# risc0/RustCrypto-elliptic-curves

Measured on AMD Instinct MI355X. Metric: k256 variable-base scalar-muls/sec, higher is better.
Workload: dtype u32

## Files before the change

__graft_entry__.py:

```python
import os
import subprocess
import sys

ROOT = os.path.dirname(os.path.abspath(__file__))
PKG = os.path.join(ROOT, "rustcrypto-elliptic-curves_amd")
for p in (ROOT, PKG):
    if p not in sys.path:
        sys.path.insert(0, p)


def build() -> None:
    env = dict(os.environ)
    env.setdefault("HIPCC", "/opt/rocm/bin/hipcc")
    subprocess.run(["make", "-j%d" % max(2, min(8, os.cpu_count() or 4)), "-C", PKG], check=True, env=env)
    oracle_dir = os.path.join(ROOT, "oracle")
    if os.path.exists(os.path.join(oracle_dir, "Makefile")):
        subprocess.run(["make", "-C", oracle_dir], check=True, env=env)
    subprocess.run(["make", "-C", os.path.join(ROOT, "tools", "ubench"), "libecpeak.so"], check=True, env=env)
    subprocess.run(["make", "-C", os.path.join(ROOT, "examples")], check=True, env=env)
    subprocess.run(["make", "-C", os.path.join(ROOT, "tests", "hosttwin")], check=True, env=env)
    subprocess.run(["make", "-j3", "-C", os.path.join(ROOT, "tests", "devtwin")], check=True, env=env)
    import ecgpu
    ecgpu.load_library()


def smoke() -> None:
    import numpy as np
    import ecgpu
    from oracle import ecmodel as M
    from oracle import synth

    ctx = ecgpu.Context(0)
    c = M.K256
    cv = ctx.curve("k256")
    n = 64
    ks = synth.scalars(c, n)
    ps = synth.points(c, n)
    sb = np.frombuffer(b"".join(M.i2b(c, k) for k in ks), dtype=np.uint8).reshape(n, 32).copy()
    pb = np.frombuffer(b"".join(M.i2b(c, x) + M.i2b(c, y) for x, y in ps), dtype=np.uint8).reshape(n, 64).copy()
    xy, inf = cv.mul(sb, pb)
    for i in range(n):
        w = M.affine_mul(c, ks[i], ps[i])
        assert bytes(xy[i]) == M.i2b(c, w[0]) + M.i2b(c, w[1]) and inf[i] == 0, f"k256 mul mismatch at {i}"
    xyz = cv.mul(sb, pb, out_format=ecgpu.PROJECTIVE, flags=ecgpu.EXACT_REFERENCE)
    for i in range(0, n, 8):
        assert bytes(xyz[i]) == M.proj_bytes(c, M.k256_mul_ref((ps[i][0], ps[i][1], 1), ks[i])), f"exact XYZ mismatch at {i}"
    ctx.close()
    print("smoke ok: k256 variable-base scalar multiplication on cuda:0 is bit-exact against the oracle")


if __name__ == "__main__":
    build()
    if len(sys.argv) > 1 and sys.argv[1] == "smoke":
        smoke()
```

rustcrypto-elliptic-curves_amd/csrc/fe_k256.hpp:

```cpp
#pragma once
#include "mp32.hpp"

namespace ecgpu {

struct FeK256 {
  static constexpr int N = 8;
  static constexpr int NBYTES = 32;
  u32 v[8];
};

namespace k256 {

static constexpr u32 C_LO = 977;

#ifdef ECGPU_K256_BRANCHFREE
#define ECGPU_K256_RARE(cond) true
#else
#define ECGPU_K256_RARE(cond) __builtin_expect((cond), 0)
#endif
#if defined(ECGPU_K256_BRANCHFREE) || defined(ECGPU_K256_EXACT_PRODUCTS)
#define ECGPU_K256_SPEC_PRODUCTS 0
#else
#define ECGPU_K256_SPEC_PRODUCTS 1
#endif

ECGPU_HD void fold_top(u32* r, u64 T) {
  const u64 m = (u64)(u32)T * C_LO + (((u64)((u32)(T >> 32) * C_LO)) << 32);
  const u64 alo = m + (T << 32);
  const u32 a2 = (u32)(T >> 32) + (alo < m ? 1u : 0u);
  u32 c = 0;
  r[0] = addc(r[0], (u32)alo, c);
  r[1] = addc(r[1], (u32)(alo >> 32), c);
  r[2] = addc(r[2], a2, c);
#pragma unroll
  for (int i = 3; i < 8; i++) r[i] = addc(r[i], 0u, c);
  u32 c2 = 0;
  r[0] = addc(r[0], c ? C_LO : 0u, c2);
  r[1] = addc(r[1], c, c2);
  r[2] = addc(r[2], 0u, c2);
}

ECGPU_HD void fold_top_fast(u32* r, u64 T) {
  const u32 t0 = (u32)T, t1 = (u32)(T >> 32);
  const u64 p = (u64)t0 * C_LO;
  const u32 s1 = (u32)(p >> 32) + t1 * C_LO;
  u32 ca = 0;
  const u32 a1 = addc(s1, t0, ca);
  const u32 a2 = t1 + ca;
  u32 c = 0;
  r[0] = addc(r[0], (u32)p, c);
  r[1] = addc(r[1], a1, c);
  r[2] = addc(r[2], a2, c);
  if (ECGPU_K256_RARE(c != 0)) {
#pragma unroll
    for (int i = 3; i < 8; i++) r[i] = addc(r[i], 0u, c);
    u32 c2 = 0;
    r[0] = addc(r[0], c ? C_LO : 0u, c2);
    r[1] = addc(r[1], c, c2);
    r[2] = addc(r[2], 0u, c2);
  }
}

namespace nc_bound {
using u128 = unsigned __int128;
constexpr u128 MAX_PRODUCT = (u128)0xFFFFFFFFu * 0xFFFFFFFFu;
static_assert(17 * MAX_PRODUCT + ((u128)1 << 37) < ((u128)1 << 69), "a column with a carry-in < 2^37 sums to < 2^69: it pops < 2^37");
static_assert(((u128)1 << 37) + (u128)0xFFFFFFFFu * C_LO < ((u128)1 << 43), "fold product on a popped carry: < 2^43, no carry");
static_assert(((u128)1 << 37) + 0xFFFFFFFFu < ((u128)1 << 64), "s_i * d_8 on a popped carry: no carry");
static_assert((u128)0xFFFFFFFFu + MAX_PRODUCT < ((u128)1 << 64), "s_0 * d_8 then one product on a zeroed accumulator: no carry");
}
template <int K>
ECGPU_HD void mul_high_column(u32* h, Acc96& c, const u32* a, const u32* b) {
  mac_product_column<8, K, 0, true, (K == 8 ? 1 : 0)>(c, a, b, nullptr, nullptr);
  h[K - 8] = acc_pop(c);
}
template <int K>
ECGPU_HD void mul_low_column(u32* t, Acc96& c, const u32* a, const u32* b, const u32* h) {
  const u32 xa[1] = {h[K]}, xb[1] = {C_LO};
  mac_product_column<8, K, 1, true, 1>(c, a, b, xa, xb);
  t[K] = acc_pop(c);
}
ECGPU_HD void mul_exact(FeK256& r, const FeK256& a, const FeK256& b) {
  u32 h[8], t[8];
  Acc96 c{0, 0};
  mul_high_column<8>(h, c, a.v, b.v);  mul_high_column<9>(h, c, a.v, b.v);
  mul_high_column<10>(h, c, a.v, b.v); mul_high_column<11>(h, c, a.v, b.v);
  mul_high_column<12>(h, c, a.v, b.v); mul_high_column<13>(h, c, a.v, b.v);
  mul_high_column<14>(h, c, a.v, b.v);
  h[7] = (u32)c.lo;
  c.lo = 0; c.hi = 0;
  mul_low_column<0>(t, c, a.v, b.v, h); mul_low_column<1>(t, c, a.v, b.v, h);
  mul_low_column<2>(t, c, a.v, b.v, h); mul_low_column<3>(t, c, a.v, b.v, h);
  mul_low_column<4>(t, c, a.v, b.v, h); mul_low_column<5>(t, c, a.v, b.v, h);
  mul_low_column<6>(t, c, a.v, b.v, h); mul_low_column<7>(t, c, a.v, b.v, h);
  u32 cy = 0;
  r.v[0] = t[0];
#pragma unroll
  for (int i = 1; i < 8; i++) r.v[i] = addc(t[i], h[i - 1], cy);
  const u64 T = c.lo + h[7] + cy;
  fold_top_fast(r.v, T);
}

namespace nc_bound {
constexpr u128 high_carry_in(int K) {
  u128 c = 0;
  for (int k = 8; k < K; k++) c = (c + (u128)(15 - k) * MAX_PRODUCT) >> 32;
  return c;
}
static_assert(high_carry_in(14) + MAX_PRODUCT < ((u128)1 << 64), "mul, high column 14: a_7 b_7 on the popped carry cannot carry");
static_assert(2 * high_carry_in(14) + 1 + MAX_PRODUCT >= ((u128)1 << 64), "with two products per column (mul_add2) it can: speculative there");
static_assert(((u128)1 << 43) + MAX_PRODUCT >= ((u128)1 << 64) && MAX_PRODUCT == ((u128)1 << 64) - ((u128)1 << 33) + 1,
              "low half: the speculative product starts below 2^43 and carries only for a product above 2^64 - 2^43");
static_assert(((u128)1 << 37) + 0xFFFFFFFFu < ((u128)1 << 38), "high half: the speculative product starts below 2^38 (popped carry, + s_i d_8 in mul_add_sqr)");
}
#if !ECGPU_K256_SPEC_PRODUCTS
ECGPU_HD void mul(FeK256& r, const FeK256& a, const FeK256& b) { mul_exact(r, a, b); }
#else
template <int K>
ECGPU_HD void mul_high_column_spec(u32* h, Acc96& c, const u32* a, const u32* b, u64& raised) {
  static_assert(K >= 9 && K <= 14, "column 8 starts from zero and stays mul_high_column<8>");
  if constexpr (K == 14) {
    mac_nc(c, a[7], b[7]);
    h[6] = (u32)c.lo;
    c.lo >>= 32;
    return;
  } else {
    u64 k = 0;
    mac_product_column<8, K, 0, true, 0, true>(c, a, b, nullptr, nullptr, k);
    ECGPU_SPEC_NOTE("mul", K, k != 0);
    raised |= k;
  }
  h[K - 8] = acc_pop(c);
}
template <int K>
ECGPU_HD void mul_low_column_spec(u32* t, Acc96& c, const u32* a, const u32* b, const u32* h, u64& raised) {
  static_assert(K >= 1 && K <= 7, "column 0 has one product after the fold term, whose carry addition creates c.hi: it stays mul_low_column<0>");
  const u32 xa[1] = {h[K]}, xb[1] = {C_LO};
  u64 k = 0;
  mac_product_column<8, K, 1, true, 1, true>(c, a, b, xa, xb, k);
  ECGPU_SPEC_NOTE("mul", K, k != 0);
  raised |= k;
  t[K] = acc_pop(c);
}
ECGPU_HD void mul_finish(FeK256& r, const u32* t, const u32* h, const Acc96& c, u32 h8) {
  u32 cy = 0;
  r.v[0] = t[0];
#pragma unroll
  for (int i = 1; i < 8; i++) r.v[i] = addc(t[i], h[i - 1], cy);
  const u64 T = c.lo + h[7] + cy + (((u64)h8 << 32) | (h8 ? C_LO : 0u));
  fold_top_fast(r.v, T);
}
ECGPU_HD void mul(FeK256& r, const FeK256& a, const FeK256& b) {
  u32 h[8], t[8];
  u64 raised = 0;
  Acc96 c{0, 0};
  mul_high_column<8>(h, c, a.v, b.v);
  mul_high_column_spec<9>(h, c, a.v, b.v, raised);  mul_high_column_spec<10>(h, c, a.v, b.v, raised);
  mul_high_column_spec<11>(h, c, a.v, b.v, raised); mul_high_column_spec<12>(h, c, a.v, b.v, raised);
  mul_high_column_spec<13>(h, c, a.v, b.v, raised); mul_high_column_spec<14>(h, c, a.v, b.v, raised);
  h[7] = (u32)c.lo;
  c.lo = 0; c.hi = 0;
  mul_low_column<0>(t, c, a.v, b.v, h); mul_low_column_spec<1>(t, c, a.v, b.v, h, raised);
  mul_low_column_spec<2>(t, c, a.v, b.v, h, raised); mul_low_column_spec<3>(t, c, a.v, b.v, h, raised);
  mul_low_column_spec<4>(t, c, a.v, b.v, h, raised); mul_low_column_spec<5>(t, c, a.v, b.v, h, raised);
  mul_low_column_spec<6>(t, c, a.v, b.v, h, raised); mul_low_column_spec<7>(t, c, a.v, b.v, h, raised);
  mul_finish(r, t, h, c, 0);
}
#endif

template <int K>
ECGPU_HD void mul2_high_column(u32* h, Acc96& c, const u32* a, const u32* b, const u32* e, const u32* f) {
  mac_product_column<8, K, 0, true, (K == 8 ? 1 : 0)>(c, a, b, nullptr, nullptr);
  mac_product_column<8, K, 0, false>(c, e, f, nullptr, nullptr);
  h[K - 8] = acc_pop(c);
}
template <int K>
ECGPU_HD void mul2_low_column(u32* t, Acc96& c, const u32* a, const u32* b, const u32* e, const u32* f, const u32* h) {
  const u32 xa[1] = {h[K]}, xb[1] = {C_LO};
  mac_product_column<8, K, 1, true, 1>(c, a, b, xa, xb);
  mac_product_column<8, K, 0, false>(c, e, f, nullptr, nullptr);
  t[K] = acc_pop(c);
}
ECGPU_HD void mul_add2_exact(FeK256& r, const FeK256& a, const FeK256& b, const FeK256& e, const FeK256& f) {
  u32 h[8], t[8];
  Acc96 c{0, 0};
  mul2_high_column<8>(h, c, a.v, b.v, e.v, f.v);  mul2_high_column<9>(h, c, a.v, b.v, e.v, f.v);
  mul2_high_column<10>(h, c, a.v, b.v, e.v, f.v); mul2_high_column<11>(h, c, a.v, b.v, e.v, f.v);
  mul2_high_column<12>(h, c, a.v, b.v, e.v, f.v); mul2_high_column<13>(h, c, a.v, b.v, e.v, f.v);
  mul2_high_column<14>(h, c, a.v, b.v, e.v, f.v);
  h[7] = (u32)c.lo;
  const u32 h8 = (u32)(c.lo >> 32);
  c.lo = 0; c.hi = 0;
  mul2_low_column<0>(t, c, a.v, b.v, e.v, f.v, h); mul2_low_column<1>(t, c, a.v, b.v, e.v, f.v, h);
  mul2_low_column<2>(t, c, a.v, b.v, e.v, f.v, h); mul2_low_column<3>(t, c, a.v, b.v, e.v, f.v, h);
  mul2_low_column<4>(t, c, a.v, b.v, e.v, f.v, h); mul2_low_column<5>(t, c, a.v, b.v, e.v, f.v, h);
  mul2_low_column<6>(t, c, a.v, b.v, e.v, f.v, h); mul2_low_column<7>(t, c, a.v, b.v, e.v, f.v, h);
  u32 cy = 0;
  r.v[0] = t[0];
#pragma unroll
  for (int i = 1; i < 8; i++) r.v[i] = addc(t[i], h[i - 1], cy);
  const u64 T = c.lo + h[7] + cy + (((u64)h8 << 32) | (h8 ? C_LO : 0u));
  fold_top_fast(r.v, T);
}

#if !ECGPU_K256_SPEC_PRODUCTS
ECGPU_HD void mul_add2(FeK256& r, const FeK256& a, const FeK256& b, const FeK256& e, const FeK256& f) { mul_add2_exact(r, a, b, e, f); }
#else
template <int K>
ECGPU_HD void mul2_high_column_spec(u32* h, Acc96& c, const u32* a, const u32* b, const u32* e, const u32* f, u64& raised) {
  static_assert(K >= 9 && K <= 13, "column 8 starts from zero; column 14 has one product a_7 b_7, whose carry addition creates c.hi");
  u64 k = 0;
  mac_product_column<8, K, 0, true, 0, true>(c, a, b, nullptr, nullptr, k);
  ECGPU_SPEC_NOTE("mul_add2", K, k != 0);
  raised |= k;
  mac_product_column<8, K, 0, false>(c, e, f, nullptr, nullptr);
  h[K - 8] = acc_pop(c);
}
template <int K>
ECGPU_HD void mul2_low_column_spec(u32* t, Acc96& c, const u32* a, const u32* b, const u32* e, const u32* f, const u32* h, u64& raised) {
  static_assert(K >= 1 && K <= 7, "column 0 stays mul2_low_column<0>, as in mul");
  const u32 xa[1] = {h[K]}, xb[1] = {C_LO};
  u64 k = 0;
  mac_product_column<8, K, 1, true, 1, true>(c, a, b, xa, xb, k);
  ECGPU_SPEC_NOTE("mul_add2", K, k != 0);
  raised |= k;
  mac_product_column<8, K, 0, false>(c, e, f, nullptr, nullptr);
  t[K] = acc_pop(c);
}
ECGPU_HD void mul_add2(FeK256& r, const FeK256& a, const FeK256& b, const FeK256& e, const FeK256& f) {
  u32 h[8], t[8];
  u64 raised = 0;
  Acc96 c{0, 0};
  mul2_high_column<8>(h, c, a.v, b.v, e.v, f.v);
  mul2_high_column_spec<9>(h, c, a.v, b.v, e.v, f.v, raised);  mul2_high_column_spec<10>(h, c, a.v, b.v, e.v, f.v, raised);
  mul2_high_column_spec<11>(h, c, a.v, b.v, e.v, f.v, raised); mul2_high_column_spec<12>(h, c, a.v, b.v, e.v, f.v, raised);
  mul2_high_column_spec<13>(h, c, a.v, b.v, e.v, f.v, raised); mul2_high_column<14>(h, c, a.v, b.v, e.v, f.v);
  h[7] = (u32)c.lo;
  const u32 h8 = (u32)(c.lo >> 32);
  c.lo = 0; c.hi = 0;
  mul2_low_column<0>(t, c, a.v, b.v, e.v, f.v, h); mul2_low_column_spec<1>(t, c, a.v, b.v, e.v, f.v, h, raised);
  mul2_low_column_spec<2>(t, c, a.v, b.v, e.v, f.v, h, raised); mul2_low_column_spec<3>(t, c, a.v, b.v, e.v, f.v, h, raised);
  mul2_low_column_spec<4>(t, c, a.v, b.v, e.v, f.v, h, raised); mul2_low_column_spec<5>(t, c, a.v, b.v, e.v, f.v, h, raised);
  mul2_low_column_spec<6>(t, c, a.v, b.v, e.v, f.v, h, raised); mul2_low_column_spec<7>(t, c, a.v, b.v, e.v, f.v, h, raised);
  mul_finish(r, t, h, c, h8);
}
#endif

constexpr int sqr2_terms(int K) {
  int m = 0;
  if (K % 2 == 1 && (K - 1) / 2 <= 6) m++;
  if (K % 2 == 0 && K / 2 <= 7) m++;
  for (int i = 0; i <= 6; i++)
    if (K - i >= i + 2 && K - i <= 8) m++;
  return m;
}
constexpr bool sqr2_has_d8(int K) { return K >= 8 && K <= 14; }
template <int K>
ECGPU_HD void sqr2_column_terms(u32* pa, u32* pb, const u32* s, const u32* e, const u32* d) {
  int m = 0;
  if constexpr (K % 2 == 1 && (K - 1) / 2 <= 6) { pa[m] = s[(K - 1) / 2]; pb[m] = e[(K + 1) / 2]; m++; }
  if constexpr (K % 2 == 0 && K / 2 <= 7) { pa[m] = s[K / 2]; pb[m] = s[K / 2]; m++; }
#pragma unroll
  for (int i = 0; i <= 6; i++)
    if (K - i >= i + 2 && K - i <= 7) { pa[m] = s[i]; pb[m] = d[K - i]; m++; }
}
ECGPU_HD void sqr2_operands(u32* e, u32* d, const u32* s) {
#pragma unroll
  for (int j = 1; j < 8; j++) e[j] = s[j] << 1;
#pragma unroll
  for (int j = 2; j < 8; j++) d[j] = (s[j] << 1) | (s[j - 1] >> 31);
  d[8] = s[7] >> 31;
}
template <int K, int NX, bool FRESH, int NC>
ECGPU_HD void mulsq_column(Acc96& c, const u32* a, const u32* b, const u32* s, const u32* e, const u32* d, const u32* xa, const u32* xb) {
  constexpr int LO = (K - 7) > 0 ? (K - 7) : 0;
  constexpr int HI = K < 7 ? K : 7;
  constexpr int M = HI - LO + 1;
  constexpr int MS = sqr2_terms(K);
  constexpr int D8 = sqr2_has_d8(K) ? 1 : 0;
  u32 pa[M + MS + NX + 1], pb[M + MS + NX + 1];
#pragma unroll
  for (int m = 0; m < NX; m++) { pa[m] = xa[m]; pb[m] = xb[m]; }
  if constexpr (D8) { pa[NX] = s[K - 8]; pb[NX] = d[8]; }
#pragma unroll
  for (int m = 0; m < M; m++) { pa[NX + D8 + m] = a[LO + m]; pb[NX + D8 + m] = b[K - LO - m]; }
  sqr2_column_terms<K>(pa + NX + D8 + M, pb + NX + D8 + M, s, e, d);
  mac_cols<M + MS + NX, FRESH, NC>(c, pa, pb);
}
template <int K>
ECGPU_HD void mulsq_high_column(u32* h, Acc96& c, const u32* a, const u32* b, const u32* s, const u32* e, const u32* d) {
  static_assert(sqr2_has_d8(K), "every high column has its d_8 term");
  mulsq_column<K, 0, true, (K == 8 ? 2 : 1)>(c, a, b, s, e, d, nullptr, nullptr);
  h[K - 8] = acc_pop(c);
}
template <int K>
ECGPU_HD void mulsq_low_column(u32* t, Acc96& c, const u32* a, const u32* b, const u32* s, const u32* e, const u32* d, const u32* h) {
  const u32 xa[1] = {h[K]}, xb[1] = {C_LO};
  mulsq_column<K, 1, true, 1>(c, a, b, s, e, d, xa, xb);
  t[K] = acc_pop(c);
}
ECGPU_HD void mul_add_sqr_exact(FeK256& r, const FeK256& a, const FeK256& b, const FeK256& s) {
  u32 e[8], d[9], h[8], t[8];
  e[0] = 0; d[0] = 0; d[1] = 0;
  sqr2_operands(e, d, s.v);
  Acc96 c{0, 0};
  mulsq_high_column<8>(h, c, a.v, b.v, s.v, e, d);  mulsq_high_column<9>(h, c, a.v, b.v, s.v, e, d);
  mulsq_high_column<10>(h, c, a.v, b.v, s.v, e, d); mulsq_high_column<11>(h, c, a.v, b.v, s.v, e, d);
  mulsq_high_column<12>(h, c, a.v, b.v, s.v, e, d); mulsq_high_column<13>(h, c, a.v, b.v, s.v, e, d);
  mulsq_high_column<14>(h, c, a.v, b.v, s.v, e, d);
  h[7] = (u32)c.lo;
  const u32 h8 = (u32)(c.lo >> 32);
  c.lo = 0; c.hi = 0;
  mulsq_low_column<0>(t, c, a.v, b.v, s.v, e, d, h); mulsq_low_column<1>(t, c, a.v, b.v, s.v, e, d, h);
  mulsq_low_column<2>(t, c, a.v, b.v, s.v, e, d, h); mulsq_low_column<3>(t, c, a.v, b.v, s.v, e, d, h);
  mulsq_low_column<4>(t, c, a.v, b.v, s.v, e, d, h); mulsq_low_column<5>(t, c, a.v, b.v, s.v, e, d, h);
  mulsq_low_column<6>(t, c, a.v, b.v, s.v, e, d, h); mulsq_low_column<7>(t, c, a.v, b.v, s.v, e, d, h);
  u32 cy = 0;
  r.v[0] = t[0];
#pragma unroll
  for (int i = 1; i < 8; i++) r.v[i] = addc(t[i], h[i - 1], cy);
  const u64 T = c.lo + h[7] + cy + (((u64)h8 << 32) | (h8 ? C_LO : 0u));
  fold_top_fast(r.v, T);
}

#if !ECGPU_K256_SPEC_PRODUCTS
ECGPU_HD void mul_add_sqr(FeK256& r, const FeK256& a, const FeK256& b, const FeK256& s) { mul_add_sqr_exact(r, a, b, s); }
#else
template <int K, int NX, int NC>
ECGPU_HD void mulsq_column_spec(Acc96& c, const u32* a, const u32* b, const u32* s, const u32* e, const u32* d, const u32* xa, const u32* xb, u64& raised) {
  constexpr int LO = (K - 7) > 0 ? (K - 7) : 0;
  constexpr int HI = K < 7 ? K : 7;
  constexpr int M = HI - LO + 1;
  constexpr int MS = sqr2_terms(K);
  constexpr int D8 = sqr2_has_d8(K) ? 1 : 0;
  u32 pa[M + MS + NX + 1], pb[M + MS + NX + 1];
#pragma unroll
  for (int m = 0; m < NX; m++) { pa[m] = xa[m]; pb[m] = xb[m]; }
  if constexpr (D8) { pa[NX] = s[K - 8]; pb[NX] = d[8]; }
#pragma unroll
  for (int m = 0; m < M; m++) { pa[NX + D8 + m] = a[LO + m]; pb[NX + D8 + m] = b[K - LO - m]; }
  sqr2_column_terms<K>(pa + NX + D8 + M, pb + NX + D8 + M, s, e, d);
  u64 k = 0;
  mac_cols<M + MS + NX, true, NC, true>(c, pa, pb, k);
  ECGPU_SPEC_NOTE("mul_add_sqr", K, k != 0);
  raised |= k;
}
template <int K>
ECGPU_HD void mulsq_high_column_spec(u32* h, Acc96& c, const u32* a, const u32* b, const u32* s, const u32* e, const u32* d, u64& raised) {
  static_assert(K >= 9 && K <= 14, "column 8 starts from zero and stays mulsq_high_column<8>");
  mulsq_column_spec<K, 0, 1>(c, a, b, s, e, d, nullptr, nullptr, raised);
  h[K - 8] = acc_pop(c);
}
template <int K>
ECGPU_HD void mulsq_low_column_spec(u32* t, Acc96& c, const u32* a, const u32* b, const u32* s, const u32* e, const u32* d, const u32* h, u64& raised) {
  const u32 xa[1] = {h[K]}, xb[1] = {C_LO};
  mulsq_column_spec<K, 1, 1>(c, a, b, s, e, d, xa, xb, raised);
  t[K] = acc_pop(c);
}
ECGPU_HD void mul_add_sqr(FeK256& r, const FeK256& a, const FeK256& b, const FeK256& s) {
  u32 e[8], d[9], h[8], t[8];
  e[0] = 0; d[0] = 0; d[1] = 0;
  sqr2_operands(e, d, s.v);
  u64 raised = 0;
  Acc96 c{0, 0};
  mulsq_high_column<8>(h, c, a.v, b.v, s.v, e, d);
  mulsq_high_column_spec<9>(h, c, a.v, b.v, s.v, e, d, raised);  mulsq_high_column_spec<10>(h, c, a.v, b.v, s.v, e, d, raised);
  mulsq_high_column_spec<11>(h, c, a.v, b.v, s.v, e, d, raised); mulsq_high_column_spec<12>(h, c, a.v, b.v, s.v, e, d, raised);
  mulsq_high_column_spec<13>(h, c, a.v, b.v, s.v, e, d, raised); mulsq_high_column_spec<14>(h, c, a.v, b.v, s.v, e, d, raised);
  h[7] = (u32)c.lo;
  const u32 h8 = (u32)(c.lo >> 32);
  c.lo = 0; c.hi = 0;
  mulsq_low_column_spec<0>(t, c, a.v, b.v, s.v, e, d, h, raised); mulsq_low_column_spec<1>(t, c, a.v, b.v, s.v, e, d, h, raised);
  mulsq_low_column_spec<2>(t, c, a.v, b.v, s.v, e, d, h, raised); mulsq_low_column_spec<3>(t, c, a.v, b.v, s.v, e, d, h, raised);
  mulsq_low_column_spec<4>(t, c, a.v, b.v, s.v, e, d, h, raised); mulsq_low_column_spec<5>(t, c, a.v, b.v, s.v, e, d, h, raised);
  mulsq_low_column_spec<6>(t, c, a.v, b.v, s.v, e, d, h, raised); mulsq_low_column_spec<7>(t, c, a.v, b.v, s.v, e, d, h, raised);
  mul_finish(r, t, h, c, h8);
}
#endif

ECGPU_HD void reduce16(FeK256& r, const u32* w) {
  u32 u[8];
  u64 acc = 0;
#pragma unroll
  for (int k = 0; k < 8; k++) {
    acc = (u64)w[8 + k] * C_LO + (acc >> 32);
    u[k] = (u32)acc;
  }
  u32 c1 = 0, c2 = 0;
  u32 t[8];
#pragma unroll
  for (int k = 0; k < 8; k++) t[k] = addc(w[k], u[k], c1);
  r.v[0] = t[0];
#pragma unroll
  for (int k = 1; k < 8; k++) r.v[k] = addc(t[k], w[8 + k - 1], c2);
  const u64 T = (acc >> 32) + c1 + c2 + w[15];
  fold_top_fast(r.v, T);
}

ECGPU_HD void sqr_exact(FeK256& r, const FeK256& a) {
  u32 w[16];
  mp_sqr_wide<8>(w, a.v);
  reduce16(r, w);
}

ECGPU_HD void sqr(FeK256& r, const FeK256& a) {
#if !ECGPU_K256_SPEC_PRODUCTS
  sqr_exact(r, a);
#else
  u32 w[16];
  u64 raised = 0;
  mp_sqr_wide<8, true>(w, a.v, raised);
  reduce16(r, w);
#endif
}

ECGPU_HD void add(FeK256& r, const FeK256& a, const FeK256& b) {
  const u32 c = mp_add<8>(r.v, a.v, b.v);
  u32 c2 = 0;
  r.v[0] = addc(r.v[0], c ? C_LO : 0u, c2);
  r.v[1] = addc(r.v[1], c, c2);
  if (ECGPU_K256_RARE(c2 != 0)) {
#pragma unroll
    for (int i = 2; i < 8; i++) r.v[i] = addc(r.v[i], 0u, c2);
    u32 c3 = 0;
    r.v[0] = addc(r.v[0], c2 ? C_LO : 0u, c3);
    r.v[1] = addc(r.v[1], c2, c3);
  }
}

ECGPU_HD void sub(FeK256& r, const FeK256& a, const FeK256& b) {
  const u32 bw = mp_sub<8>(r.v, a.v, b.v);
  u32 b2 = 0;
  r.v[0] = subb(r.v[0], bw ? C_LO : 0u, b2);
  r.v[1] = subb(r.v[1], bw, b2);
  if (ECGPU_K256_RARE(b2 != 0)) {
#pragma unroll
    for (int i = 2; i < 8; i++) r.v[i] = subb(r.v[i], 0u, b2);
    u32 b3 = 0;
    r.v[0] = subb(r.v[0], b2 ? C_LO : 0u, b3);
    r.v[1] = subb(r.v[1], b2, b3);
  }
}

ECGPU_HD void sub2(FeK256& r, const FeK256& a, const FeK256& b, const FeK256& c) {
  const u32 w = mp_sub<8>(r.v, a.v, b.v) + mp_sub<8>(r.v, r.v, c.v);
  u32 b2 = 0;
  r.v[0] = subb(r.v[0], w * C_LO, b2);
  r.v[1] = subb(r.v[1], w, b2);
  if (ECGPU_K256_RARE(b2 != 0)) {
#pragma unroll
    for (int i = 2; i < 8; i++) r.v[i] = subb(r.v[i], 0u, b2);
    u32 b3 = 0;
    r.v[0] = subb(r.v[0], b2 ? C_LO : 0u, b3);
    r.v[1] = subb(r.v[1], b2, b3);
  }
}

ECGPU_HD void half(FeK256& r, const FeK256& a) {
  const u32 m = 0u - (a.v[0] & 1u);
  u32 t[8], c = 0;
  t[0] = addc(a.v[0], m & (0u - C_LO), c);
  t[1] = addc(a.v[1], m & 0xFFFFFFFEu, c);
#pragma unroll
  for (int i = 2; i < 8; i++) t[i] = addc(a.v[i], m, c);
#pragma unroll
  for (int i = 0; i < 7; i++) r.v[i] = (t[i] >> 1) | (t[i + 1] << 31);
  r.v[7] = (t[7] >> 1) | (c << 31);
}

ECGPU_HD void set_zero(FeK256& r) { mp_zero<8>(r.v); }
ECGPU_HD void set_one(FeK256& r) { mp_zero<8>(r.v); r.v[0] = 1; }
ECGPU_HD void set_u32(FeK256& r, u32 x) { mp_zero<8>(r.v); r.v[0] = x; }

ECGPU_HD void neg(FeK256& r, const FeK256& a) {
  FeK256 z;
  set_zero(z);
  sub(r, z, a);
}
ECGPU_HD void dbl(FeK256& r, const FeK256& a) { add(r, a, a); }

template <int K>
ECGPU_HD void shl(FeK256& r, const FeK256& a) {
  static_assert(K >= 1 && K <= 3, "small shifts only");
  const u32 top = a.v[7] >> (32 - K);
  u32 t[8];
#pragma unroll
  for (int i = 7; i >= 1; i--) t[i] = (a.v[i] << K) | (a.v[i - 1] >> (32 - K));
  t[0] = a.v[0] << K;
  u32 c = 0;
  r.v[0] = addc(t[0], top * C_LO, c);
  r.v[1] = addc(t[1], top, c);
#pragma unroll
  for (int i = 2; i < 8; i++) r.v[i] = t[i];
  if (ECGPU_K256_RARE(c != 0)) {
// ... 115 lines not shown
```

rustcrypto-elliptic-curves_amd/csrc/mp32.hpp:

```cpp
#pragma once
#include <stdint.h>

#if defined(__HIPCC__)
#include <hip/hip_runtime.h>
#define ECGPU_HD __host__ __device__ __forceinline__
#else
#define ECGPU_HD inline
#endif

#if defined(__HIP_DEVICE_COMPILE__)
#define ECGPU_ASM 1
#else
#define ECGPU_ASM 0
#endif

#ifndef ECGPU_TABLE_TOUCH
#define ECGPU_TABLE_TOUCH(idx) ((void)0)
#endif
#ifndef ECGPU_EXC_NOTE
#define ECGPU_EXC_NOTE(site, cond) ((void)0)
#endif
#ifndef ECGPU_SPEC_NOTE
#define ECGPU_SPEC_NOTE(site, column, raised) ((void)0)
#endif
// ... 76 lines not shown
template <int N>
ECGPU_HD void mp_select(u32* r, bool cond, const u32* a, const u32* b) {
#pragma unroll
  for (int i = 0; i < N; i++) r[i] = cond ? a[i] : b[i];
}

struct Acc96 {
  u64 lo;
  u32 hi;
};

ECGPU_HD void mac(Acc96& c, u32 a, u32 b) {
#if ECGPU_ASM
  asm("v_mad_u64_u32 %0, vcc, %2, %3, %0\n\tv_addc_co_u32 %1, vcc, 0, %1, vcc"
      : "+v"(c.lo), "+v"(c.hi)
      : "v"(a), "v"(b)
      : "vcc");
#else
  u64 p = (u64)a * b;
  c.lo += p;
  c.hi += (c.lo < p);
#endif
}
ECGPU_HD void mac_nc(Acc96& c, u32 a, u32 b) { c.lo += (u64)a * b; }
ECGPU_HD u64 mac_spec(Acc96& c, u32 a, u32 b) {
  const u64 p = (u64)a * b;
  c.lo += p;
  return c.lo < p ? 1u : 0u;
}
ECGPU_HD void mac_spec_fix(Acc96& c, u64 k) {
#if ECGPU_ASM
  asm("v_addc_co_u32 %0, vcc, 0, %0, %1" : "+v"(c.hi) : "s"(k) : "vcc");
#else
  c.hi += (u32)k;
#endif
}
ECGPU_HD void acc_sub32(Acc96& c, u32 w) {
  u32 l0 = (u32)c.lo, l1 = (u32)(c.lo >> 32), bw = 0;
  l0 = subb(l0, w, bw);
  l1 = subb(l1, 0u, bw);
  c.hi = subb(c.hi, 0u, bw);
  c.lo = ((u64)l1 << 32) | l0;
}

#include "mp32_cols.inc"

template <int M, bool FRESH = false, int NC = 0>
ECGPU_HD void mac_cols(Acc96& c, const u32* pa, const u32* pb) {
  static_assert(M >= 1, "column length");
  static_assert(NC >= 0 && NC <= 2 && NC <= M, "at most two leading products without a carry");
  if constexpr (M > 12) {
    mac_cols<12, FRESH, NC>(c, pa, pb);
    mac_cols<M - 12, false>(c, pa + 12, pb + 12);
  } else if constexpr (NC > 0) {
    mac_cols_nc<M, FRESH, NC>(c, pa, pb);
  } else {
    if constexpr (M == 1) { if constexpr (FRESH) mac_col1_f(c, pa[0], pb[0]); else mac_col1(c, pa[0], pb[0]); }
    if constexpr (M == 2) { if constexpr (FRESH) mac_col2_f(c, pa[0], pb[0], pa[1], pb[1]); else mac_col2(c, pa[0], pb[0], pa[1], pb[1]); }
    if constexpr (M == 3) { if constexpr (FRESH) mac_col3_f(c, pa[0], pb[0], pa[1], pb[1], pa[2], pb[2]); else mac_col3(c, pa[0], pb[0], pa[1], pb[1], pa[2], pb[2]); }
    if constexpr (M == 4) { if constexpr (FRESH) mac_col4_f(c, pa[0], pb[0], pa[1], pb[1], pa[2], pb[2], pa[3], pb[3]); else mac_col4(c, pa[0], pb[0], pa[1], pb[1], pa[2], pb[2], pa[3], pb[3]); }
    if constexpr (M == 5) { if constexpr (FRESH) mac_col5_f(c, pa[0], pb[0], pa[1], pb[1], pa[2], pb[2], pa[3], pb[3], pa[4], pb[4]); else mac_col5(c, pa[0], pb[0], pa[1], pb[1], pa[2], pb[2], pa[3], pb[3], pa[4], pb[4]); }
    if constexpr (M == 6) { if constexpr (FRESH) mac_col6_f(c, pa[0], pb[0], pa[1], pb[1], pa[2], pb[2], pa[3], pb[3], pa[4], pb[4], pa[5], pb[5]); else mac_col6(c, pa[0], pb[0], pa[1], pb[1], pa[2], pb[2], pa[3], pb[3], pa[4], pb[4], pa[5], pb[5]); }
    if constexpr (M == 7) { if constexpr (FRESH) mac_col7_f(c, pa[0], pb[0], pa[1], pb[1], pa[2], pb[2], pa[3], pb[3], pa[4], pb[4], pa[5], pb[5], pa[6], pb[6]); else mac_col7(c, pa[0], pb[0], pa[1], pb[1], pa[2], pb[2], pa[3], pb[3], pa[4], pb[4], pa[5], pb[5], pa[6], pb[6]); }
    if constexpr (M == 8) { if constexpr (FRESH) mac_col8_f(c, pa[0], pb[0], pa[1], pb[1], pa[2], pb[2], pa[3], pb[3], pa[4], pb[4], pa[5], pb[5], pa[6], pb[6], pa[7], pb[7]); else mac_col8(c, pa[0], pb[0], pa[1], pb[1], pa[2], pb[2], pa[3], pb[3], pa[4], pb[4], pa[5], pb[5], pa[6], pb[6], pa[7], pb[7]); }
    if constexpr (M == 9) { if constexpr (FRESH) mac_col9_f(c, pa[0], pb[0], pa[1], pb[1], pa[2], pb[2], pa[3], pb[3], pa[4], pb[4], pa[5], pb[5], pa[6], pb[6], pa[7], pb[7], pa[8], pb[8]); else mac_col9(c, pa[0], pb[0], pa[1], pb[1], pa[2], pb[2], pa[3], pb[3], pa[4], pb[4], pa[5], pb[5], pa[6], pb[6], pa[7], pb[7], pa[8], pb[8]); }
    if constexpr (M == 10) { if constexpr (FRESH) mac_col10_f(c, pa[0], pb[0], pa[1], pb[1], pa[2], pb[2], pa[3], pb[3], pa[4], pb[4], pa[5], pb[5], pa[6], pb[6], pa[7], pb[7], pa[8], pb[8], pa[9], pb[9]); else mac_col10(c, pa[0], pb[0], pa[1], pb[1], pa[2], pb[2], pa[3], pb[3], pa[4], pb[4], pa[5], pb[5], pa[6], pb[6], pa[7], pb[7], pa[8], pb[8], pa[9], pb[9]); }
    if constexpr (M == 11) { if constexpr (FRESH) mac_col11_f(c, pa[0], pb[0], pa[1], pb[1], pa[2], pb[2], pa[3], pb[3], pa[4], pb[4], pa[5], pb[5], pa[6], pb[6], pa[7], pb[7], pa[8], pb[8], pa[9], pb[9], pa[10], pb[10]); else mac_col11(c, pa[0], pb[0], pa[1], pb[1], pa[2], pb[2], pa[3], pb[3], pa[4], pb[4], pa[5], pb[5], pa[6], pb[6], pa[7], pb[7], pa[8], pb[8], pa[9], pb[9], pa[10], pb[10]); }
    if constexpr (M == 12) { if constexpr (FRESH) mac_col12_f(c, pa[0], pb[0], pa[1], pb[1], pa[2], pb[2], pa[3], pb[3], pa[4], pb[4], pa[5], pb[5], pa[6], pb[6], pa[7], pb[7], pa[8], pb[8], pa[9], pb[9], pa[10], pb[10], pa[11], pb[11]); else mac_col12(c, pa[0], pb[0], pa[1], pb[1], pa[2], pb[2], pa[3], pb[3], pa[4], pb[4], pa[5], pb[5], pa[6], pb[6], pa[7], pb[7], pa[8], pb[8], pa[9], pb[9], pa[10], pb[10], pa[11], pb[11]); }
  }
}
template <int M, bool FRESH = false, int NC = 0, bool SPEC = false>
ECGPU_HD void mac_cols(Acc96& c, const u32* pa, const u32* pb, u64& raised) {
  if constexpr (!SPEC) {
    mac_cols<M, FRESH, NC>(c, pa, pb);
  } else {
    static_assert(M >= 1 && NC >= 0 && NC <= 2 && NC + 1 <= M, "the speculative product follows the no-carry products");
    u64 k;
    if constexpr (M > 12) {
      mac_cols_s1<12, FRESH, NC>(c, k, pa, pb);
      mac_cols<M - 12, false>(c, pa + 12, pb + 12);
    } else {
      mac_cols_s1<M, FRESH, NC>(c, k, pa, pb);
    }
    if (__builtin_expect(k != 0, 0)) mac_spec_fix(c, k);
    raised |= k;
  }
}
template <int N, int K, int NX, bool FRESH = false, int NC = 0>
ECGPU_HD void mac_product_column(Acc96& c, const u32* a, const u32* b, const u32* xa, const u32* xb) {
  constexpr int LO = (K - (N - 1)) > 0 ? (K - (N - 1)) : 0;
  constexpr int HI = K < (N - 1) ? K : (N - 1);
  constexpr int M = HI - LO + 1;
  u32 pa[M + NX + 1], pb[M + NX + 1];
#pragma unroll
  for (int m = 0; m < NX; m++) { pa[m] = xa[m]; pb[m] = xb[m]; }
#pragma unroll
  for (int m = 0; m < M; m++) { pa[NX + m] = a[LO + m]; pb[NX + m] = b[K - LO - m]; }
  mac_cols<M + NX, FRESH, NC>(c, pa, pb);
}
template <int N, int K, int NX, bool FRESH = false, int NC = 0, bool SPEC = false>
ECGPU_HD void mac_product_column(Acc96& c, const u32* a, const u32* b, const u32* xa, const u32* xb, u64& raised) {
  constexpr int LO = (K - (N - 1)) > 0 ? (K - (N - 1)) : 0;
  constexpr int HI = K < (N - 1) ? K : (N - 1);
  constexpr int M = HI - LO + 1;
  u32 pa[M + NX + 1], pb[M + NX + 1];
#pragma unroll
  for (int m = 0; m < NX; m++) { pa[m] = xa[m]; pb[m] = xb[m]; }
#pragma unroll
  for (int m = 0; m < M; m++) { pa[NX + m] = a[LO + m]; pb[NX + m] = b[K - LO - m]; }
  mac_cols<M + NX, FRESH, NC, SPEC>(c, pa, pb, raised);
}

ECGPU_HD u32 acc_pop(Acc96& c) {
  u32 r = (u32)c.lo;
  c.lo = (c.lo >> 32) | ((u64)c.hi << 32);
  c.hi = 0;
  return r;
}

ECGPU_HD u32 acc_pop_signed(Acc96& c) {
  u32 r = (u32)c.lo;
  c.lo = (c.lo >> 32) | ((u64)c.hi << 32);
  c.hi = (u32)((int32_t)c.hi >> 31);
  return r;
}

template <int N>
ECGPU_HD void mp_mul_wide(u32* r, const u32* a, const u32* b) {
  Acc96 c{0, 0};
#pragma unroll
  for (int k = 0; k < 2 * N - 1; k++) {
#pragma unroll
    for (int i = 0; i < N; i++) {
      const int j = k - i;
      if (j >= 0 && j < N) {
        if (k == 0 || k == 2 * N - 2) mac_nc(c, a[i], b[j]); else mac(c, a[i], b[j]);
      }
    }
    r[k] = acc_pop(c);
  }
  r[2 * N - 1] = (u32)c.lo;
}


template <int N, int K>
ECGPU_HD void mac_cross_column(Acc96& c, const u32* a) {
  constexpr int LO = (K - (N - 1)) > 0 ? (K - (N - 1)) : 0;
  constexpr int HI = (K - 1) / 2;
  constexpr int M = HI - LO + 1;
  if constexpr (M >= 1) {
    u32 pa[M], pb[M];
#pragma unroll
    for (int m = 0; m < M; m++) { pa[m] = a[LO + m]; pb[m] = a[K - LO - m]; }
    mac_cols<M, true>(c, pa, pb);
  }
}
template <int N, int K>
ECGPU_HD void sqr_cross_columns(u32* x, Acc96& c, const u32* a) {
  if constexpr (K < 2 * N - 2) {
    mac_cross_column<N, K>(c, a);
    x[K] = acc_pop(c);
    sqr_cross_columns<N, K + 1>(x, c, a);
  }
}

template <int N>
constexpr bool sqr_cross_first_nc(int K) {
  typedef unsigned __int128 u128;
  const u128 maxp = (u128)0xFFFFFFFFu * 0xFFFFFFFFu;
  u128 c = 0;
  for (int k = 1; k < K; k++) {
    const int lo = (k - (N - 1)) > 0 ? (k - (N - 1)) : 0, hi = (k - 1) / 2;
    c = (c + (u128)(hi - lo + 1) * maxp) >> 32;
  }
  return c + maxp < ((u128)1 << 64);
}
static_assert(sqr_cross_first_nc<8>(1) && sqr_cross_first_nc<8>(2) && sqr_cross_first_nc<8>(3) && sqr_cross_first_nc<8>(4) && sqr_cross_first_nc<8>(5) &&
              !sqr_cross_first_nc<8>(6) && !sqr_cross_first_nc<8>(10) && sqr_cross_first_nc<8>(11) && sqr_cross_first_nc<8>(12) && sqr_cross_first_nc<8>(13),
              "the carry-free cross columns of the 8-word square, as the comments and tests/k256_spec_carry_vectors.py list them");
template <int N, int K, bool SPEC>
ECGPU_HD void mac_cross_column(Acc96& c, const u32* a, u64& raised) {
  constexpr int LO = (K - (N - 1)) > 0 ? (K - (N - 1)) : 0;
  constexpr int HI = (K - 1) / 2;
  constexpr int M = HI - LO + 1;
  if constexpr (M >= 1) {
    u32 pa[M], pb[M];
#pragma unroll
    for (int m = 0; m < M; m++) { pa[m] = a[LO + m]; pb[m] = a[K - LO - m]; }
    if constexpr (SPEC && M == 1 && sqr_cross_first_nc<N>(K)) mac_nc(c, pa[0], pb[0]);
    else if constexpr (SPEC && M >= 2 && sqr_cross_first_nc<N>(K)) mac_cols<M, true, 1>(c, pa, pb);
    else mac_cols<M, true, 0, (SPEC && M >= 2)>(c, pa, pb, raised);
  }
}
template <int N, int K, bool SPEC>
ECGPU_HD void sqr_cross_columns(u32* x, Acc96& c, const u32* a, u64& raised) {
  if constexpr (K < 2 * N - 2) {
    u64 k = 0;
    mac_cross_column<N, K, SPEC>(c, a, k);
    if constexpr (SPEC && (K - 1) / 2 - ((K - (N - 1)) > 0 ? (K - (N - 1)) : 0) + 1 >= 2 && !sqr_cross_first_nc<N>(K)) { ECGPU_SPEC_NOTE("sqr", K, k != 0); }
    raised |= k;
    x[K] = acc_pop(c);
    sqr_cross_columns<N, K + 1, SPEC>(x, c, a, raised);
  }
}

template <int N>
ECGPU_HD void mp_sqr_wide(u32* r, const u32* a) {
  u32 x[2 * N];
  Acc96 c{0, 0};
  x[0] = 0;
  sqr_cross_columns<N, 1>(x, c, a);
  x[2 * N - 2] = (u32)c.lo;
  x[2 * N - 1] = (u32)(c.lo >> 32);
  u32 carry = 0;
#pragma unroll
  for (int i = 0; i < N; i++) {
    const u64 d = (u64)a[i] * a[i];
    const u32 lo2 = (x[2 * i] << 1) | (i ? (x[2 * i - 1] >> 31) : 0);
    const u32 hi2 = (x[2 * i + 1] << 1) | (x[2 * i] >> 31);
    r[2 * i] = addc(lo2, (u32)d, carry);
    r[2 * i + 1] = addc(hi2, (u32)(d >> 32), carry);
  }
}
template <int N, bool SPEC>
ECGPU_HD void mp_sqr_wide(u32* r, const u32* a, u64& raised) {
  u32 x[2 * N];
  Acc96 c{0, 0};
  x[0] = 0;
  sqr_cross_columns<N, 1, SPEC>(x, c, a, raised);
  x[2 * N - 2] = (u32)c.lo;
  x[2 * N - 1] = (u32)(c.lo >> 32);
  u32 carry = 0;
#pragma unroll
  for (int i = 0; i < N; i++) {
    const u64 d = (u64)a[i] * a[i];
    const u32 lo2 = (x[2 * i] << 1) | (i ? (x[2 * i - 1] >> 31) : 0);
    const u32 hi2 = (x[2 * i + 1] << 1) | (x[2 * i] >> 31);
    r[2 * i] = addc(lo2, (u32)d, carry);
    r[2 * i + 1] = addc(hi2, (u32)(d >> 32), carry);
  }
}

ECGPU_HD u32 bswap32(u32 x) { return __builtin_bswap32(x); }

}
```

Before: 160.2 million.

## Replace per-column speculative carry fixups with whole-product recompute on rare miss

Previously each speculative product column tested its raised-carry mask and applied mac_spec_fix inline. Now each multiply, multiply-add and square first runs all columns without fixups. If any column raised a carry, it reruns the whole product with fixups enabled, and the rare branch is marked with probability 1.0 so it is laid out cold. This removes per-column branches and fixup code from the hot path, in exchange for a full recompute on a mispredicted carry and larger code.

Measured after the change: 161.6 million, median of 6. No clear change (+0.9%).

```diff
diff --git a/__graft_entry__.py b/__graft_entry__.py
--- a/__graft_entry__.py
+++ b/__graft_entry__.py
@@ -20,6 +20,7 @@
     subprocess.run(["make", "-C", os.path.join(ROOT, "examples")], check=True, env=env)
     subprocess.run(["make", "-C", os.path.join(ROOT, "tests", "hosttwin")], check=True, env=env)
     subprocess.run(["make", "-j3", "-C", os.path.join(ROOT, "tests", "devtwin")], check=True, env=env)
+    subprocess.run(["make", "-j2", "-C", os.path.join(ROOT, "tests", "devtwin_alias")], check=True, env=env)
     import ecgpu
     ecgpu.load_library()
 
diff --git a/rustcrypto-elliptic-curves_amd/csrc/fe_k256.hpp b/rustcrypto-elliptic-curves_amd/csrc/fe_k256.hpp
--- a/rustcrypto-elliptic-curves_amd/csrc/fe_k256.hpp
+++ b/rustcrypto-elliptic-curves_amd/csrc/fe_k256.hpp
@@ -15,8 +15,10 @@
 
 #ifdef ECGPU_K256_BRANCHFREE
 #define ECGPU_K256_RARE(cond) true
+#elif defined(ECGPU_K256_EXACT_PRODUCTS)
+#define ECGPU_K256_RARE(cond) __builtin_expect((cond), 0)
 #else
-#define ECGPU_K256_RARE(cond) __builtin_expect((cond), 0)
+#define ECGPU_K256_RARE(cond) __builtin_expect_with_probability((cond), 0, 1.0)
 #endif
 #if defined(ECGPU_K256_BRANCHFREE) || defined(ECGPU_K256_EXACT_PRODUCTS)
 #define ECGPU_K256_SPEC_PRODUCTS 0
@@ -116,7 +118,7 @@
 #if !ECGPU_K256_SPEC_PRODUCTS
 ECGPU_HD void mul(FeK256& r, const FeK256& a, const FeK256& b) { mul_exact(r, a, b); }
 #else
-template <int K>
+template <int K, bool FIX>
 ECGPU_HD void mul_high_column_spec(u32* h, Acc96& c, const u32* a, const u32* b, u64& raised) {
   static_assert(K >= 9 && K <= 14, "column 8 starts from zero and stays mul_high_column<8>");
   if constexpr (K == 14) {
@@ -127,44 +129,52 @@
   } else {
     u64 k = 0;
     mac_product_column<8, K, 0, true, 0, true>(c, a, b, nullptr, nullptr, k);
-    ECGPU_SPEC_NOTE("mul", K, k != 0);
+    if constexpr (FIX) mac_spec_fix(c, k);
+    ECGPU_SPEC_NOTE("mul", K, (FIX || raised == 0) && k != 0);
     raised |= k;
   }
   h[K - 8] = acc_pop(c);
 }
-template <int K>
+template <int K, bool FIX>
 ECGPU_HD void mul_low_column_spec(u32* t, Acc96& c, const u32* a, const u32* b, const u32* h, u64& raised) {
   static_assert(K >= 1 && K <= 7, "column 0 has one product after the fold term, whose carry addition creates c.hi: it stays mul_low_column<0>");
   const u32 xa[1] = {h[K]}, xb[1] = {C_LO};
   u64 k = 0;
   mac_product_column<8, K, 1, true, 1, true>(c, a, b, xa, xb, k);
-  ECGPU_SPEC_NOTE("mul", K, k != 0);
+  if constexpr (FIX) mac_spec_fix(c, k);
+  ECGPU_SPEC_NOTE("mul", K, (FIX || raised == 0) && k != 0);
   raised |= k;
   t[K] = acc_pop(c);
 }
-ECGPU_HD void mul_finish(FeK256& r, const u32* t, const u32* h, const Acc96& c, u32 h8) {
+template <bool FIX>
+ECGPU_HD void mul_columns(u32* t, u32* h, Acc96& c, const u32* a, const u32* b, u64& raised) {
+  c.lo = 0; c.hi = 0;
+  mul_high_column<8>(h, c, a, b);
+  mul_high_column_spec<9, FIX>(h, c, a, b, raised);  mul_high_column_spec<10, FIX>(h, c, a, b, raised);
+  mul_high_column_spec<11, FIX>(h, c, a, b, raised); mul_high_column_spec<12, FIX>(h, c, a, b, raised);
+  mul_high_column_spec<13, FIX>(h, c, a, b, raised); mul_high_column_spec<14, FIX>(h, c, a, b, raised);
+  h[7] = (u32)c.lo;
+  c.lo = 0; c.hi = 0;
+  mul_low_column<0>(t, c, a, b, h); mul_low_column_spec<1, FIX>(t, c, a, b, h, raised);
+  mul_low_column_spec<2, FIX>(t, c, a, b, h, raised); mul_low_column_spec<3, FIX>(t, c, a, b, h, raised);
+  mul_low_column_spec<4, FIX>(t, c, a, b, h, raised); mul_low_column_spec<5, FIX>(t, c, a, b, h, raised);
+  mul_low_column_spec<6, FIX>(t, c, a, b, h, raised); mul_low_column_spec<7, FIX>(t, c, a, b, h, raised);
+}
+ECGPU_HD void mul_finish(FeK256& r, const u32* t, const u32* h, const Acc96& c, u64 top) {
   u32 cy = 0;
   r.v[0] = t[0];
 #pragma unroll
   for (int i = 1; i < 8; i++) r.v[i] = addc(t[i], h[i - 1], cy);
-  const u64 T = c.lo + h[7] + cy + (((u64)h8 << 32) | (h8 ? C_LO : 0u));
+  const u64 T = c.lo + top + cy + ((top >> 32) ? C_LO : 0u);
   fold_top_fast(r.v, T);
 }
 ECGPU_HD void mul(FeK256& r, const FeK256& a, const FeK256& b) {
   u32 h[8], t[8];
   u64 raised = 0;
-  Acc96 c{0, 0};
-  mul_high_column<8>(h, c, a.v, b.v);
-  mul_high_column_spec<9>(h, c, a.v, b.v, raised);  mul_high_column_spec<10>(h, c, a.v, b.v, raised);
-  mul_high_column_spec<11>(h, c, a.v, b.v, raised); mul_high_column_spec<12>(h, c, a.v, b.v, raised);
-  mul_high_column_spec<13>(h, c, a.v, b.v, raised); mul_high_column_spec<14>(h, c, a.v, b.v, raised);
-  h[7] = (u32)c.lo;
-  c.lo = 0; c.hi = 0;
-  mul_low_column<0>(t, c, a.v, b.v, h); mul_low_column_spec<1>(t, c, a.v, b.v, h, raised);
-  mul_low_column_spec<2>(t, c, a.v, b.v, h, raised); mul_low_column_spec<3>(t, c, a.v, b.v, h, raised);
-  mul_low_column_spec<4>(t, c, a.v, b.v, h, raised); mul_low_column_spec<5>(t, c, a.v, b.v, h, raised);
-  mul_low_column_spec<6>(t, c, a.v, b.v, h, raised); mul_low_column_spec<7>(t, c, a.v, b.v, h, raised);
-  mul_finish(r, t, h, c, 0);
+  Acc96 c;
+  mul_columns<false>(t, h, c, a.v, b.v, raised);
+  if (ECGPU_K256_RARE(raised != 0)) mul_columns<true>(t, h, c, a.v, b.v, raised);
+  mul_finish(r, t, h, c, h[7]);
 }
 #endif
 
@@ -206,43 +216,51 @@
 #if !ECGPU_K256_SPEC_PRODUCTS
 ECGPU_HD void mul_add2(FeK256& r, const FeK256& a, const FeK256& b, const FeK256& e, const FeK256& f) { mul_add2_exact(r, a, b, e, f); }
 #else
-template <int K>
+template <int K, bool FIX>
 ECGPU_HD void mul2_high_column_spec(u32* h, Acc96& c, const u32* a, const u32* b, const u32* e, const u32* f, u64& raised) {
   static_assert(K >= 9 && K <= 13, "column 8 starts from zero; column 14 has one product a_7 b_7, whose carry addition creates c.hi");
   u64 k = 0;
   mac_product_column<8, K, 0, true, 0, true>(c, a, b, nullptr, nullptr, k);
-  ECGPU_SPEC_NOTE("mul_add2", K, k != 0);
+  if constexpr (FIX) mac_spec_fix(c, k);
+  ECGPU_SPEC_NOTE("mul_add2", K, (FIX || raised == 0) && k != 0);
   raised |= k;
   mac_product_column<8, K, 0, false>(c, e, f, nullptr, nullptr);
   h[K - 8] = acc_pop(c);
 }
-template <int K>
+template <int K, bool FIX>
 ECGPU_HD void mul2_low_column_spec(u32* t, Acc96& c, const u32* a, const u32* b, const u32* e, const u32* f, const u32* h, u64& raised) {
   static_assert(K >= 1 && K <= 7, "column 0 stays mul2_low_column<0>, as in mul");
   const u32 xa[1] = {h[K]}, xb[1] = {C_LO};
   u64 k = 0;
   mac_product_column<8, K, 1, true, 1, true>(c, a, b, xa, xb, k);
-  ECGPU_SPEC_NOTE("mul_add2", K, k != 0);
+  if constexpr (FIX) mac_spec_fix(c, k);
+  ECGPU_SPEC_NOTE("mul_add2", K, (FIX || raised == 0) && k != 0);
   raised |= k;
   mac_product_column<8, K, 0, false>(c, e, f, nullptr, nullptr);
   t[K] = acc_pop(c);
 }
+template <bool FIX>
+ECGPU_HD void mul2_columns(u32* t, u32* h, Acc96& c, u64& top, const u32* a, const u32* b, const u32* e, const u32* f, u64& raised) {
+  c.lo = 0; c.hi = 0;
+  mul2_high_column<8>(h, c, a, b, e, f);
+  mul2_high_column_spec<9, FIX>(h, c, a, b, e, f, raised);  mul2_high_column_spec<10, FIX>(h, c, a, b, e, f, raised);
+  mul2_high_column_spec<11, FIX>(h, c, a, b, e, f, raised); mul2_high_column_spec<12, FIX>(h, c, a, b, e, f, raised);
+  mul2_high_column_spec<13, FIX>(h, c, a, b, e, f, raised); mul2_high_column<14>(h, c, a, b, e, f);
+  top = c.lo;
+  h[7] = (u32)top;
+  c.lo = 0; c.hi = 0;
+  mul2_low_column<0>(t, c, a, b, e, f, h); mul2_low_column_spec<1, FIX>(t, c, a, b, e, f, h, raised);
+  mul2_low_column_spec<2, FIX>(t, c, a, b, e, f, h, raised); mul2_low_column_spec<3, FIX>(t, c, a, b, e, f, h, raised);
+  mul2_low_column_spec<4, FIX>(t, c, a, b, e, f, h, raised); mul2_low_column_spec<5, FIX>(t, c, a, b, e, f, h, raised);
+  mul2_low_column_spec<6, FIX>(t, c, a, b, e, f, h, raised); mul2_low_column_spec<7, FIX>(t, c, a, b, e, f, h, raised);
+}
 ECGPU_HD void mul_add2(FeK256& r, const FeK256& a, const FeK256& b, const FeK256& e, const FeK256& f) {
   u32 h[8], t[8];
-  u64 raised = 0;
-  Acc96 c{0, 0};
-  mul2_high_column<8>(h, c, a.v, b.v, e.v, f.v);
-  mul2_high_column_spec<9>(h, c, a.v, b.v, e.v, f.v, raised);  mul2_high_column_spec<10>(h, c, a.v, b.v, e.v, f.v, raised);
-  mul2_high_column_spec<11>(h, c, a.v, b.v, e.v, f.v, raised); mul2_high_column_spec<12>(h, c, a.v, b.v, e.v, f.v, raised);
-  mul2_high_column_spec<13>(h, c, a.v, b.v, e.v, f.v, raised); mul2_high_column<14>(h, c, a.v, b.v, e.v, f.v);
-  h[7] = (u32)c.lo;
-  const u32 h8 = (u32)(c.lo >> 32);
-  c.lo = 0; c.hi = 0;
-  mul2_low_column<0>(t, c, a.v, b.v, e.v, f.v, h); mul2_low_column_spec<1>(t, c, a.v, b.v, e.v, f.v, h, raised);
-  mul2_low_column_spec<2>(t, c, a.v, b.v, e.v, f.v, h, raised); mul2_low_column_spec<3>(t, c, a.v, b.v, e.v, f.v, h, raised);
-  mul2_low_column_spec<4>(t, c, a.v, b.v, e.v, f.v, h, raised); mul2_low_column_spec<5>(t, c, a.v, b.v, e.v, f.v, h, raised);
-  mul2_low_column_spec<6>(t, c, a.v, b.v, e.v, f.v, h, raised); mul2_low_column_spec<7>(t, c, a.v, b.v, e.v, f.v, h, raised);
-  mul_finish(r, t, h, c, h8);
+  u64 raised = 0, top;
+  Acc96 c;
+  mul2_columns<false>(t, h, c, top, a.v, b.v, e.v, f.v, raised);
+  if (ECGPU_K256_RARE(raised != 0)) mul2_columns<true>(t, h, c, top, a.v, b.v, e.v, f.v, raised);
+  mul_finish(r, t, h, c, top);
 }
 #endif
 
@@ -326,7 +344,7 @@
 #if !ECGPU_K256_SPEC_PRODUCTS
 ECGPU_HD void mul_add_sqr(FeK256& r, const FeK256& a, const FeK256& b, const FeK256& s) { mul_add_sqr_exact(r, a, b, s); }
 #else
-template <int K, int NX, int NC>
+template <int K, int NX, int NC, bool FIX>
 ECGPU_HD void mulsq_column_spec(Acc96& c, const u32* a, const u32* b, const u32* s, const u32* e, const u32* d, const u32* xa, const u32* xb, u64& raised) {
   constexpr int LO = (K - 7) > 0 ? (K - 7) : 0;
   constexpr int HI = K < 7 ? K : 7;
@@ -342,39 +360,46 @@
   sqr2_column_terms<K>(pa + NX + D8 + M, pb + NX + D8 + M, s, e, d);
   u64 k = 0;
   mac_cols<M + MS + NX, true, NC, true>(c, pa, pb, k);
-  ECGPU_SPEC_NOTE("mul_add_sqr", K, k != 0);
+  if constexpr (FIX) mac_spec_fix(c, k);
+  ECGPU_SPEC_NOTE("mul_add_sqr", K, (FIX || raised == 0) && k != 0);
   raised |= k;
 }
-template <int K>
+template <int K, bool FIX>
 ECGPU_HD void mulsq_high_column_spec(u32* h, Acc96& c, const u32* a, const u32* b, const u32* s, const u32* e, const u32* d, u64& raised) {
   static_assert(K >= 9 && K <= 14, "column 8 starts from zero and stays mulsq_high_column<8>");
-  mulsq_column_spec<K, 0, 1>(c, a, b, s, e, d, nullptr, nullptr, raised);
+  mulsq_column_spec<K, 0, 1, FIX>(c, a, b, s, e, d, nullptr, nullptr, raised);
   h[K - 8] = acc_pop(c);
 }
-template <int K>
+template <int K, bool FIX>
 ECGPU_HD void mulsq_low_column_spec(u32* t, Acc96& c, const u32* a, const u32* b, const u32* s, const u32* e, const u32* d, const u32* h, u64& raised) {
   const u32 xa[1] = {h[K]}, xb[1] = {C_LO};
-  mulsq_column_spec<K, 1, 1>(c, a, b, s, e, d, xa, xb, raised);
+  mulsq_column_spec<K, 1, 1, FIX>(c, a, b, s, e, d, xa, xb, raised);
   t[K] = acc_pop(c);
+}
+template <bool FIX>
+ECGPU_HD void mulsq_columns(u32* t, u32* h, Acc96& c, u64& top, const u32* a, const u32* b, const u32* s, const u32* e, const u32* d, u64& raised) {
+  c.lo = 0; c.hi = 0;
+  mulsq_high_column<8>(h, c, a, b, s, e, d);
+  mulsq_high_column_spec<9, FIX>(h, c, a, b, s, e, d, raised);  mulsq_high_column_spec<10, FIX>(h, c, a, b, s, e, d, raised);
+  mulsq_high_column_spec<11, FIX>(h, c, a, b, s, e, d, raised); mulsq_high_column_spec<12, FIX>(h, c, a, b, s, e, d, raised);
+  mulsq_high_column_spec<13, FIX>(h, c, a, b, s, e, d, raised); mulsq_high_column_spec<14, FIX>(h, c, a, b, s, e, d, raised);
+  top = c.lo;
+  h[7] = (u32)top;
+  c.lo = 0; c.hi = 0;
+  mulsq_low_column_spec<0, FIX>(t, c, a, b, s, e, d, h, raised); mulsq_low_column_spec<1, FIX>(t, c, a, b, s, e, d, h, raised);
+  mulsq_low_column_spec<2, FIX>(t, c, a, b, s, e, d, h, raised); mulsq_low_column_spec<3, FIX>(t, c, a, b, s, e, d, h, raised);
+  mulsq_low_column_spec<4, FIX>(t, c, a, b, s, e, d, h, raised); mulsq_low_column_spec<5, FIX>(t, c, a, b, s, e, d, h, raised);
+  mulsq_low_column_spec<6, FIX>(t, c, a, b, s, e, d, h, raised); mulsq_low_column_spec<7, FIX>(t, c, a, b, s, e, d, h, raised);
 }
 ECGPU_HD void mul_add_sqr(FeK256& r, const FeK256& a, const FeK256& b, const FeK256& s) {
   u32 e[8], d[9], h[8], t[8];
   e[0] = 0; d[0] = 0; d[1] = 0;
   sqr2_operands(e, d, s.v);
-  u64 raised = 0;
-  Acc96 c{0, 0};
-  mulsq_high_column<8>(h, c, a.v, b.v, s.v, e, d);
-  mulsq_high_column_spec<9>(h, c, a.v, b.v, s.v, e, d, raised);  mulsq_high_column_spec<10>(h, c, a.v, b.v, s.v, e, d, raised);
-  mulsq_high_column_spec<11>(h, c, a.v, b.v, s.v, e, d, raised); mulsq_high_column_spec<12>(h, c, a.v, b.v, s.v, e, d, raised);
-  mulsq_high_column_spec<13>(h, c, a.v, b.v, s.v, e, d, raised); mulsq_high_column_spec<14>(h, c, a.v, b.v, s.v, e, d, raised);
-  h[7] = (u32)c.lo;
-  const u32 h8 = (u32)(c.lo >> 32);
-  c.lo = 0; c.hi = 0;
-  mulsq_low_column_spec<0>(t, c, a.v, b.v, s.v, e, d, h, raised); mulsq_low_column_spec<1>(t, c, a.v, b.v, s.v, e, d, h, raised);
-  mulsq_low_column_spec<2>(t, c, a.v, b.v, s.v, e, d, h, raised); mulsq_low_column_spec<3>(t, c, a.v, b.v, s.v, e, d, h, raised);
-  mulsq_low_column_spec<4>(t, c, a.v, b.v, s.v, e, d, h, raised); mulsq_low_column_spec<5>(t, c, a.v, b.v, s.v, e, d, h, raised);
-  mulsq_low_column_spec<6>(t, c, a.v, b.v, s.v, e, d, h, raised); mulsq_low_column_spec<7>(t, c, a.v, b.v, s.v, e, d, h, raised);
-  mul_finish(r, t, h, c, h8);
+  u64 raised = 0, top;
+  Acc96 c;
+  mulsq_columns<false>(t, h, c, top, a.v, b.v, s.v, e, d, raised);
+  if (ECGPU_K256_RARE(raised != 0)) mulsq_columns<true>(t, h, c, top, a.v, b.v, s.v, e, d, raised);
+  mul_finish(r, t, h, c, top);
 }
 #endif
 
@@ -407,9 +432,11 @@
 #if !ECGPU_K256_SPEC_PRODUCTS
   sqr_exact(r, a);
 #else
-  u32 w[16];
+  u32 x[16], w[16];
   u64 raised = 0;
-  mp_sqr_wide<8, true>(w, a.v, raised);
+  mp_sqr_cross<8, true, false>(x, a.v, raised);
+  if (ECGPU_K256_RARE(raised != 0)) mp_sqr_cross<8, true, true>(x, a.v, raised);
+  mp_sqr_finish<8>(w, x, a.v);
   reduce16(r, w);
 #endif
 }
diff --git a/rustcrypto-elliptic-curves_amd/csrc/mp32.hpp b/rustcrypto-elliptic-curves_amd/csrc/mp32.hpp
--- a/rustcrypto-elliptic-curves_amd/csrc/mp32.hpp
+++ b/rustcrypto-elliptic-curves_amd/csrc/mp32.hpp
@@ -182,7 +182,6 @@
     } else {
       mac_cols_s1<M, FRESH, NC>(c, k, pa, pb);
     }
-    if (__builtin_expect(k != 0, 0)) mac_spec_fix(c, k);
     raised |= k;
   }
 }
@@ -292,15 +291,18 @@
     else mac_cols<M, true, 0, (SPEC && M >= 2)>(c, pa, pb, raised);
   }
 }
-template <int N, int K, bool SPEC>
+template <int N, int K, bool SPEC, bool FIX = false>
 ECGPU_HD void sqr_cross_columns(u32* x, Acc96& c, const u32* a, u64& raised) {
   if constexpr (K < 2 * N - 2) {
     u64 k = 0;
     mac_cross_column<N, K, SPEC>(c, a, k);
-    if constexpr (SPEC && (K - 1) / 2 - ((K - (N - 1)) > 0 ? (K - (N - 1)) : 0) + 1 >= 2 && !sqr_cross_first_nc<N>(K)) { ECGPU_SPEC_NOTE("sqr", K, k != 0); }
+    if constexpr (SPEC && (K - 1) / 2 - ((K - (N - 1)) > 0 ? (K - (N - 1)) : 0) + 1 >= 2 && !sqr_cross_first_nc<N>(K)) {
+      if constexpr (FIX) mac_spec_fix(c, k);
+      ECGPU_SPEC_NOTE("sqr", K, (FIX || raised == 0) && k != 0);
+    }
     raised |= k;
     x[K] = acc_pop(c);
-    sqr_cross_columns<N, K + 1, SPEC>(x, c, a, raised);
+    sqr_cross_columns<N, K + 1, SPEC, FIX>(x, c, a, raised);
   }
 }
 
@@ -322,14 +324,16 @@
     r[2 * i + 1] = addc(hi2, (u32)(d >> 32), carry);
   }
 }
-template <int N, bool SPEC>
-ECGPU_HD void mp_sqr_wide(u32* r, const u32* a, u64& raised) {
-  u32 x[2 * N];
+template <int N, bool SPEC, bool FIX>
+ECGPU_HD void mp_sqr_cross(u32* x, const u32* a, u64& raised) {
   Acc96 c{0, 0};
   x[0] = 0;
-  sqr_cross_columns<N, 1, SPEC>(x, c, a, raised);
+  sqr_cross_columns<N, 1, SPEC, FIX>(x, c, a, raised);
   x[2 * N - 2] = (u32)c.lo;
   x[2 * N - 1] = (u32)(c.lo >> 32);
+}
+template <int N>
+ECGPU_HD void mp_sqr_finish(u32* r, const u32* x, const u32* a) {
   u32 carry = 0;
 #pragma unroll
   for (int i = 0; i < N; i++) {
```
